# MiloszKrajewski/lz4net

Measured on AMD Instinct MI355X. Metric: uncompressed GB/s, batched 64KiB-block encode+decode: value = decode (known output size) per step over the whole resident batch; fast encode and LZ4HC encode of the same data in roofline_encode / roofline_hc, higher is better.
Workload: dtype u8

## Files before the change

### lz4net_amd/csrc/lz4hip_decode_lane4.hpp

```cpp
#pragma once
#include "lz4hip_common.hpp"
#include <type_traits>

#ifndef LZ4HIP_ITERATION_HOOK
#define LZ4HIP_ITERATION_HOOK(lane) ((void)0)
#endif
#ifndef LZ4HIP_STAT
#define LZ4HIP_STAT(slot, cond) ((void)0)
#endif
#ifdef LZ4HIP_SECTION_MARKERS
#define LZ4HIP_SECTION(name) asm volatile("; @@SECTION " name)
#elif !defined(LZ4HIP_SECTION)
#define LZ4HIP_SECTION(name) ((void)0)
#endif
#ifndef LZ4HIP_SECTION_BEGIN
#define LZ4HIP_SECTION_BEGIN() ((void)0)
#define LZ4HIP_SECTION_END(lane) ((void)0)
#endif

namespace lz4hip {

#if defined(__HIP_DEVICE_COMPILE__)
#define L4_MOV(...) wv::mov_mask(__VA_ARGS__)
#define L4_MOV8(m_, d_, a_, b_)                                                                                          \
    do {                                                                                                                 \
        wv::u32x2 p0_ = { (d_)[0], (d_)[1] }, p1_ = { (d_)[2], (d_)[3] }, p2_ = { (d_)[4], (d_)[5] }, p3_ = { (d_)[6], (d_)[7] }; \
        wv::mov2_mask(m_, p0_, wv::u32x2{ (a_).x, (a_).y }, p1_, wv::u32x2{ (a_).z, (a_).w }, p2_, wv::u32x2{ (b_).x, (b_).y }, p3_, wv::u32x2{ (b_).z, (b_).w }); \
        (d_)[0] = p0_.x; (d_)[1] = p0_.y; (d_)[2] = p1_.x; (d_)[3] = p1_.y; (d_)[4] = p2_.x; (d_)[5] = p2_.y; (d_)[6] = p3_.x; (d_)[7] = p3_.y; \
    } while (0)
#define L4_TREE_LOW(m2_, m1_, t_)                                                                                        \
    do {                                                                                                                 \
        wv::u32x2 p0_ = { (t_)[0], (t_)[1] }, p1_ = { (t_)[2], (t_)[3] }, p2_ = { (t_)[4], (t_)[5] }, p3_ = { (t_)[6], (t_)[7] }; \
        wv::mov2_mask(m2_, p0_, p1_, p1_, p2_, p2_, p3_);                                                                \
        wv::shift_dword_mask(m1_, p0_, p1_, p2_);                                                                        \
        (t_)[0] = p0_.x; (t_)[1] = p0_.y; (t_)[2] = p1_.x; (t_)[3] = p1_.y; (t_)[4] = p2_.x;                             \
    } while (0)
#else
LZ4HIP_DEVICE void lane4_mov_sel(wv::mask_t) {}
template <class T, class... REST>
LZ4HIP_DEVICE void lane4_mov_sel(wv::mask_t m, T& d, T s, REST&&... rest)
{
    d = (T)wv::sel(m, (uint32_t)s, (uint32_t)d);
    lane4_mov_sel(m, static_cast<REST&&>(rest)...);
}
#define L4_MOV(...) lane4_mov_sel(__VA_ARGS__)
#define L4_MOV8(m_, d_, a_, b_)                                                                                          \
    lane4_mov_sel(m_, (d_)[0], (uint32_t)(a_).x, (d_)[1], (uint32_t)(a_).y, (d_)[2], (uint32_t)(a_).z, (d_)[3], (uint32_t)(a_).w, \
                      (d_)[4], (uint32_t)(b_).x, (d_)[5], (uint32_t)(b_).y, (d_)[6], (uint32_t)(b_).z, (d_)[7], (uint32_t)(b_).w)
#define L4_TREE_LOW(m2_, m1_, t_)                                                                                        \
    do {                                                                                                                 \
// ... 37 lines not shown
    constexpr bool LS = (POL & 16) != 0;
    constexpr int kDual = (POL & 32) ? 0 : (LZ4HIP_DEC4_DUAL_STORE);
    static_assert(!LS || P == 32, "sector input feeds 32-byte pieces");
    constexpr int SK = LS ? 64 : P;
    constexpr int NW = 4 + P / 4, NL = LS ? 4 : P / 16;
    constexpr int HPR = FU / 16, RECS_PER_STORE = 64 / HPR;
    constexpr int kFlushRecs = (LZ4HIP_DEC4_FLUSH_RECS) ? (LZ4HIP_DEC4_FLUSH_RECS) : FS * RECS_PER_STORE;
    constexpr bool kLineNoWrap = R % 64 == 0;
    constexpr int kNearMax = R - 20;
    constexpr bool kMoves = WAVES == 1;
    unsigned char* const frec_base = lds + kRingBytes + (uint32_t)wave * 256u;
    auto frec = [&](int i) -> Aligned16* {
        if (kFlushRecs <= 16) return (Aligned16*)(frec_base + (uint32_t)i * 16u);
        return (Aligned16*)(frec_base + (uint32_t)(i >> 4) * kRow + (uint32_t)(i & 15) * 16u);
    };
    const uint32_t lane4 = (uint32_t)(wave * 64 + lane) << 2;

    auto ring_add = [](uint32_t a, uint32_t rows256) -> uint32_t {
        const uint32_t t = a + rows256;
        if (RPOW2) return t & (kRingBytes - 1u);
        const uint32_t u = t - kRingBytes;
        return u < t ? u : t;
    };
#define L4_RING(a) (*(uint32_t*)(lds + (a)))
#define L4_PHASE_SEL(p_) wv::alignbyte(0x07060504u, 0x03020100u, (uint32_t)(p_) & 3u)

    int skew = 0, in_total = 0;
    uint64_t src_al = 0;
    uint32_t out_limit = 0;
    int ip = 0;
    uint32_t W[NW];
    wv::u32x4 L[NL];
    int wb = -16;
    int lvalid = 0;
    int pend_a = 0, pend_b = 0;
    int op = 0, fl = 0;
    uint32_t oa = lane4;
    int kind = kK4None, rem = 0, off = 8;
    int gready = 0;
    int pv = 0, p_ll = 0, p_st = 0, p_ml = 0, p_off = 0, p_flags = 0, p_res = 0;
    uint32_t p_l0 = 0, p_l1 = 0, p_l2 = 0;
    int hdr = 0;
    uint32_t token = 0;
    int final_seen = 0, final_run = 0, result = 0, done = 0;
    int exhausted = 0;
    wv::u32x4 fa = { 0, 0, 0, 0 }, fb = { 0, 0, 0, 0 };
#if defined(LZ4HIP_DEC4_BALLAST_VALU) || defined(LZ4HIP_DEC4_BALLAST_LDS)
    uint32_t ballast = 0;
#endif
#pragma unroll
    for (int j = 0; j < NW; j++) W[j] = 0;
#pragma unroll
    for (int j = 0; j < NL; j++) L[j] = wv::u32x4{ 0, 0, 0, 0 };
    auto start_block = [&](bool act) {
        skew = (int)((uint64_t)src & (uint64_t)(SK - 1));
        src_al = (uint64_t)src - (uint64_t)skew;
        in_total = iend > 0 ? (int)(((int64_t)skew + iend + P - 1) & ~(int64_t)(P - 1)) : 0;
        out_limit = oend > kLastLiterals ? (uint32_t)(oend - kLastLiterals) : 0u;
        ip = 0; wb = -16 - P; lvalid = 0; pend_a = 0; pend_b = 0; op = 0; fl = 0; oa = lane4;
        kind = kK4None; rem = 0; off = 8; gready = 0;
        pv = 0; p_ll = 0; p_st = 0; p_ml = 0; p_off = 0; p_flags = 0; p_res = 0; hdr = 0; token = 0;
        final_seen = 0; final_run = 0; result = 0; done = 0;
        if (!act || (!KNOWN && iend == 0)) { done = 1; final_seen = 1; }
    };
    start_block(active);
    LZ4HIP_SECTION_BEGIN();

#define L4_STORE2(OFF_, v_) do { const uint32_t w_ = (v_); wv::lds_store_drop<OFF_>(lds, kLdsBytes, oa, w_); wv::lds_store_drop<OFF_>(lds, kLdsBytes, ob_, w_); } while (0)
#define L4_APPEND(d0_, d1_, d2_, d3_, n_, FOUR_)                                                         \
    do {                                                                                                \
        const uint32_t sb_ = (uint32_t)op & 3u;                                                         \
        const uint32_t s_ = wv::alignbyte(0x08070605u, 0x04030201u, sb_ ^ 3u);                          \
        wv::lds_mskor(&L4_RING(oa), 0xFFFFFFFFu << (8u * sb_), wv::perm(d0_, 0u, s_));                  \
        if (kDual) {                                                                                    \
                                                    \
            const uint32_t ob_ = oa - kRingBytes;                                                       \
            const uint32_t w1_ = wv::perm(d1_, d0_, s_), w2_ = wv::perm(d2_, d1_, s_);                  \
            if (kDual == 2) {                                         \
                wv::lds_store2_rows_drop<1 * WAVES, 2 * WAVES>(lds, kLdsBytes, oa, w1_, w2_);           \
                wv::lds_store2_rows_drop<1 * WAVES, 2 * WAVES>(lds, kLdsBytes, ob_, w1_, w2_);          \
                if (FOUR_) {                                                                            \
                    const uint32_t w3_ = wv::perm(d3_, d2_, s_), w4_ = wv::perm(0u, d3_, s_);           \
                    wv::lds_store2_rows_drop<3 * WAVES, 4 * WAVES>(lds, kLdsBytes, oa, w3_, w4_);       \
                    wv::lds_store2_rows_drop<3 * WAVES, 4 * WAVES>(lds, kLdsBytes, ob_, w3_, w4_);      \
                } else {                                                                                \
                    L4_STORE2(3 * kRow, wv::perm(0u, d2_, s_));                                         \
                }                                                                                       \
            } else {                                                                                    \
                L4_STORE2(kRow, w1_);                                                                   \
                L4_STORE2(2 * kRow, w2_);                                                               \
                if (FOUR_) {                                                                            \
                    L4_STORE2(3 * kRow, wv::perm(d3_, d2_, s_));                                        \
                    L4_STORE2(4 * kRow, wv::perm(0u, d3_, s_));                                         \
                } else {                                                                                \
                    L4_STORE2(3 * kRow, wv::perm(0u, d2_, s_));                                         \
                }                                                                                       \
            }                                                                                           \
        } else {                                                                                        \
            const uint32_t a1_ = ring_add(oa, kRow), a2_ = ring_add(oa, 2 * kRow), a3_ = ring_add(oa, 3 * kRow); \
            L4_RING(a1_) = wv::perm(d1_, d0_, s_);                                                      \
            L4_RING(a2_) = wv::perm(d2_, d1_, s_);                                                      \
            if (FOUR_) {                                                                                \
                L4_RING(a3_) = wv::perm(d3_, d2_, s_);                                                  \
                L4_RING(ring_add(oa, 4 * kRow)) = wv::perm(0u, d3_, s_);                                \
            } else {                                                                                    \
                L4_RING(a3_) = wv::perm(0u, d2_, s_);                                                   \
            }                                                                                           \
        }                                                                                               \
        oa = ring_add(oa, (((sb_ + (uint32_t)(n_)) << 6) & 0x700u) * (uint32_t)WAVES);                  \
        op += (n_);                                                                                     \
    } while (0)

    auto iteration = [&](auto flush_tag, wv::u32x4& ldF, wv::u32x4& usF, int& ld_pend, int& us_pend) __attribute__((always_inline)) -> bool {
        constexpr bool FLUSH = decltype(flush_tag)::value;
        constexpr bool INPUT = IE == 1 || !FLUSH;
        constexpr int kVm = (FLUSH ? FS : 0) + 1 + (INPUT ? NL : 0);
        LZ4HIP_ITERATION_HOOK(lane);
        LZ4HIP_SECTION("T2a flush records");
        bool go = false;
        int cnt = 0;
        wv::mask_t f_act_m[FS];
        Aligned16 f_rec[FS];
        uint64_t f_g[FS];
        uint32_t f_q[FS][4];
        if constexpr (FLUSH) {
            const bool need = (done == 0) & (op - fl >= FU);
            const uint64_t needy = wv::ballot(need);
            const int cnt_all = wv::popc64(needy);
            go = cnt_all != 0;
            bool mine = false;
            if (go) {
                cnt = cnt_all < kFlushRecs ? cnt_all : kFlushRecs;
                const int frank = wv::rank_below(needy);
                mine = need & (frank < kFlushRecs);
                if (mine) {
                    const uint64_t dp = (uint64_t)dst;
                    *frec(frank) = Aligned16{ { ring_add(oa, kRingBytes - ((((uint32_t)(op - fl)) << 6) & ~0xFFu) * (uint32_t)WAVES), (uint32_t)fl, (uint32_t)dp, (uint32_t)(dp >> 32) } };
                }
                fl += mine ? FU : 0;
            }
            LZ4HIP_STAT(3, need); LZ4HIP_STAT(4, need & !mine);
        }
        LZ4HIP_SECTION("T2b record read");
        if constexpr (FLUSH) {
            if (go) wv::mem_sync();
#pragma unroll
            for (int s = 0; s < FS; s++) {
                const int idx = s * RECS_PER_STORE + lane / HPR;
                f_act_m[s] = wv::cond(idx < cnt);
                f_rec[s] = *frec(idx);
            }
        }
        LZ4HIP_SECTION("T1c near-match reads");
        const uint32_t offn = kind == kK4Near ? (uint32_t)off : 4u;
        uint32_t r0, r1, r2, r3, r4;
        {
            const uint32_t back = (((offn + 3u - ((uint32_t)op & 3u)) << 6) & ~0xFFu) * (uint32_t)WAVES;
            uint32_t sa;
            if (RPOW2) sa = (oa - back) & (kRingBytes - 1u);
            else { const uint32_t t = oa - back, u = t + kRingBytes; sa = u < t ? u : t; }
            r0 = L4_RING(sa); r1 = L4_RING(ring_add(sa, kRow)); r2 = L4_RING(ring_add(sa, 2 * kRow));
            r3 = L4_RING(ring_add(sa, 3 * kRow)); r4 = L4_RING(ring_add(sa, 4 * kRow));
        }
        LZ4HIP_SECTION("T1a window refill");
        int d = ip + skew - wb;
        {
            const bool no_more = wb + 16 + P >= in_total;
            const bool cross = (d >= P) & ((lvalid != 0) | no_more);
            const wv::mask_t cm = wv::cond(d >= P) & (wv::cond(lvalid != 0) | wv::cond(no_more));
            if constexpr (LS && kMoves) {
                const bool hi_half = ((wb + 16 + P) & 32) != 0;
                const wv::mask_t hm = wv::cond(((wb + 16 + P) & 32) != 0);
                L4_MOV(cm, W[0], W[8], W[1], W[9], W[2], W[10], W[3], W[11]);
                L4_MOV8(cm & ~hm, W + 4, L[0], L[1]);
                L4_MOV8(cm & hm, W + 4, L[2], L[3]);
                lvalid = (cross & hi_half) ? 0 : lvalid;
            } else if constexpr (LS) {
#pragma unroll
                for (int j = 0; j < 4; j++) W[j] = wv::sel(cm, W[P / 4 + j], W[j]);
                const bool hi_half = ((wb + 16 + P) & 32) != 0;
                const wv::mask_t hm = wv::cond(((wb + 16 + P) & 32) != 0);
#pragma unroll
                for (int j = 0; j < 2; j++) {
                    W[4 + 4 * j] = wv::sel(cm, wv::sel(hm, L[2 + j].x, L[j].x), W[4 + 4 * j]); W[5 + 4 * j] = wv::sel(cm, wv::sel(hm, L[2 + j].y, L[j].y), W[5 + 4 * j]);
                    W[6 + 4 * j] = wv::sel(cm, wv::sel(hm, L[2 + j].z, L[j].z), W[6 + 4 * j]); W[7 + 4 * j] = wv::sel(cm, wv::sel(hm, L[2 + j].w, L[j].w), W[7 + 4 * j]);
                }
                lvalid = (cross & hi_half) ? 0 : lvalid;
            } else {
#pragma unroll
                for (int j = 0; j < 4; j++) W[j] = wv::sel(cm, W[P / 4 + j], W[j]);
#pragma unroll
                for (int j = 0; j < NL; j++) {
                    W[4 + 4 * j] = wv::sel(cm, L[j].x, W[4 + 4 * j]); W[5 + 4 * j] = wv::sel(cm, L[j].y, W[5 + 4 * j]);
                    W[6 + 4 * j] = wv::sel(cm, L[j].z, W[6 + 4 * j]); W[7 + 4 * j] = wv::sel(cm, L[j].w, W[7 + 4 * j]);
                }
                lvalid = cross ? 0 : lvalid;
            }
            wb += cross ? P : 0;
            d -= cross ? P : 0;
        }
        LZ4HIP_SECTION("T1b cursor view (select tree + rotation)");
        const bool staged16 = d < P;
        LZ4HIP_STAT(0, true); LZ4HIP_STAT(1, done == 0); LZ4HIP_STAT(2, (done == 0) & !staged16);
        uint32_t x0, x1, x2, x3;
        {
            const uint32_t k = (uint32_t)d >> 2;
            uint32_t t[NW];
            if constexpr (kMoves && P == 32) {
                const wv::mask_t m = wv::cond((k & 4u) != 0u);
#pragma unroll
                for (int j = 0; j < 8; j++) t[j] = wv::sel(m, W[j + 4], W[j]);
                L4_TREE_LOW(wv::cond((k & 2u) != 0u), wv::cond((k & 1u) != 0u), t);
            } else {
#pragma unroll
                for (int j = 0; j < NW; j++) t[j] = W[j];
                int n = NW;
#pragma unroll
                for (int sh = P / 8; sh >= 1; sh >>= 1) {
                    const wv::mask_t m = wv::cond((k & (uint32_t)sh) != 0u);
                    n -= sh;
#pragma unroll
                    for (int j = 0; j < NW; j++)
                        if (j < n) t[j] = wv::sel(m, t[j + sh], t[j]);
                }
            }
            const uint32_t sx = L4_PHASE_SEL(d);
            x0 = wv::perm(t[1], t[0], sx); x1 = wv::perm(t[2], t[1], sx); x2 = wv::perm(t[3], t[2], sx); x3 = wv::perm(t[4], t[3], sx);
        }
        LZ4HIP_SECTION("T1c near-match source rows");
        uint32_t v0, v1, v2, v3;
        {
            const uint32_t sr = L4_PHASE_SEL((uint32_t)op - offn);
            v0 = wv::perm(r1, r0, sr); v1 = wv::perm(r2, r1, sr); v2 = wv::perm(r3, r2, sr); v3 = wv::perm(r4, r3, sr);
        }

        LZ4HIP_SECTION("T3 chunk size");
        const bool room = op - fl <= R - 46;
        const bool near = kind == kK4Near, lit = kind == kK4Lit;
        const bool can = room & (rem > 0) & !((kind == kK4Far) & (gready == 0)) & !(lit & !staged16);
        const int stride = (near & (off < 16)) ? off : 16;
        int n = can ? (rem < stride ? rem : stride) : 0;
        n = ((kind == kK4Zero) & (n > 8)) ? 8 : n;
        LZ4HIP_STAT(5, (done == 0) & (rem > 0)); LZ4HIP_STAT(6, (done == 0) & (rem > 0) & (n == 0)); LZ4HIP_STAT(7, (done == 0) & (rem > 0) & !room);
        LZ4HIP_STAT(8, (done == 0) & (rem > 0) & (kind == kK4Far) & (gready == 0)); LZ4HIP_STAT(9, (done == 0) & (rem > n));
        const int rem_after = rem - n;
        const int op_end = op + rem;

        LZ4HIP_SECTION("T2c ring rows");
        if constexpr (FLUSH) {
            const int sub = lane % HPR;
#pragma unroll
            for (int s = 0; s < FS; s++) {
                const Aligned16 r = f_rec[s];
                f_g[s] = ((uint64_t)r.w[2] | ((uint64_t)r.w[3] << 32)) + (uint64_t)(r.w[1] + 16u * (uint32_t)sub);
                const uint32_t b0 = wv::sel(f_act_m[s], ring_add(r.w[0], 4u * kRow * (uint32_t)sub), lane4);
                if (kLineNoWrap) { f_q[s][0] = L4_RING(b0); f_q[s][1] = L4_RING(b0 + kRow); f_q[s][2] = L4_RING(b0 + 2 * kRow); f_q[s][3] = L4_RING(b0 + 3 * kRow); }
                else { f_q[s][0] = L4_RING(b0); f_q[s][1] = L4_RING(ring_add(b0, kRow)); f_q[s][2] = L4_RING(ring_add(b0, 2 * kRow)); f_q[s][3] = L4_RING(ring_add(b0, 3 * kRow)); }
            }
        }

        LZ4HIP_SECTION("T4 parse ahead");
        const bool may_parse = (pv == 0) & (final_seen == 0) & !(lit & (rem > 0)) & staged16;
        LZ4HIP_STAT(10, may_parse); LZ4HIP_STAT(11, (done == 0) & (pv != 0));
        if (may_parse) {
            const uint32_t tok = hdr ? token : (x0 & 255u);
            const uint32_t t4 = tok >> 4, b1 = (x0 >> 8) & 255u, mlc = tok & 15u;
            const bool e1 = (hdr == 0) & (t4 == 15u), e2 = mlc == 15u;
            const int ll = hdr ? 0 : (int)t4 + (e1 ? (int)b1 : 0);
            const bool in_win = (hdr != 0) | (t4 <= 11u);
            const int o = hdr ? 0 : 1 + (int)t4;
            uint32_t ot;
            {
                const uint32_t q = (uint32_t)o >> 2;
                const wv::mask_t m1 = wv::cond((q & 1u) != 0u), m2 = wv::cond((q & 2u) != 0u);
                const uint32_t lo = wv::sel(m2, wv::sel(m1, x3, x2), wv::sel(m1, x1, x0));
                const uint32_t hi = wv::sel(m2, x3, wv::sel(m1, x2, x1));
                ot = wv::alignbyte(hi, lo, (uint32_t)o & 3u);
            }
            const int vo = (int)(ot & 0xFFFFu);
            const uint32_t extb = (ot >> 16) & 255u;
            const int ml = (int)mlc + kMinMatch + (e2 ? (int)extb : 0);
            const int lit_end = op_end + ll;
            const int p_after = ip + o + 2;
            bool trap = (ip + 16 > iend) | (e1 & (b1 == 255u)) | (ip + 1 + (e1 ? 1 : 0) + ll > iend);
            trap |= in_win & ((e2 & (extb == 255u)) | (vo > lit_end) | ((uint32_t)lit_end + (uint32_t)ml > out_limit));
            if (KNOWN) trap |= (hdr == 0) & (lit_end > oend - 8);
            else       trap |= ((hdr == 0) & ((lit_end > oend - kMfLimit) | (ip + 1 + (e1 ? 1 : 0) + ll > iend - 8))) | (in_win & e2 & !(p_after < iend - (kLastLiterals + 1)));
            p_l0 = wv::alignbyte(x1, x0, 1); p_l1 = wv::alignbyte(x2, x1, 1); p_l2 = wv::alignbyte(x3, x2, 1);
            token = tok;
            p_ll = in_win ? ll : 0;
            p_st = in_win ? 0 : ll;
            p_ml = in_win ? ml : 0;
            p_off = vo;
            p_flags = in_win ? 0 : (int)kF4Header;
            const int ip_fast = in_win ? p_after + (e2 ? 1 : 0) : ip + 1 + (e1 ? 1 : 0);
            if (trap) {
// ... 22 lines not shown
                        if (KNOWN && err == 0 && pos + l > iend) err = -pos;
                        p_flags = kF4Header;
                    }
                    ip = pos;
                } else {
                    int p = ip;
                    const int o_ = (int)((p < iend ? src[p] : 0u) | ((p + 1 < iend ? src[p + 1] : 0u) << 8));
                    p += 2;
                    int m = (int)(token & 15u);
                    if (m == 15) {
                        if (KNOWN) {
                            uint32_t b;
                            while ((b = (p < iend ? src[p] : 0u)) == 255) { m += 255; p++; if (m > (1 << 30)) { err = -p; break; } }
                            m += (int)b; p++;
                        } else {
                            while (p < iend - (kLastLiterals + 1)) { const uint32_t b = src[p]; p++; m += (int)b; m = m > (1 << 30) ? (1 << 30) : m; if (b != 255) break; }
                        }
                    }
                    m += kMinMatch;
                    if (err != 0) {}
                    else if (op_end - o_ < 0) err = -(ip + 2);
                    else if ((int64_t)op_end + m > (int64_t)oend - kLastLiterals) err = -p;
                    p_ll = 0; p_st = 0; p_ml = m; p_off = o_; p_flags = 0;
                    ip = p;
                    hdr = 0;
                }
                if (err != 0) { p_flags = kF4Err; p_res = err; }
                hdr = (p_flags & kF4Header) ? 1 : 0;
            } else {
                ip = ip_fast;
                hdr = in_win ? 0 : 1;
            }
            LZ4HIP_SECTION("T4 parse ahead");
            pv = 1;
        }

        LZ4HIP_SECTION("T2d flush stores");
        if constexpr (FLUSH) {
#pragma unroll
            for (int s = 0; s < FS; s++) wv::vm_store16_mask(f_act_m[s], f_g[s], f_q[s][0], f_q[s][1], f_q[s][2], f_q[s][3]);
            if (go) wv::mem_sync();
        }

        LZ4HIP_SECTION("T5 far fetch");
        {
            const wv::mask_t m_rem0 = wv::cond(rem_after == 0);
            const wv::mask_t f_cont = wv::cond(kind == kK4Far) & ~m_rem0;
            const wv::mask_t f_first = m_rem0 & wv::cond(op - fl <= R - 46) & wv::cond(pv != 0) & wv::cond(p_ml != 0) & wv::cond(p_flags == 0) & wv::cond(p_off > kNearMax);
            const int f_pos = (int)wv::sel(f_cont, (uint32_t)(op + n - off), (uint32_t)(op_end + p_ll - p_off));
            const wv::mask_t f_want = f_cont | f_first;
            const wv::mask_t f_do = f_want & wv::cond(f_pos + 16 <= fl);
            wv::vm_load16_mask<POL & 3>(f_do, (uint64_t)dst + (uint64_t)(uint32_t)f_pos, ldF);
            gready = (int)wv::sel(f_do, 1u, 0u);
            LZ4HIP_STAT(15, gready != 0); LZ4HIP_STAT(16, wv::sel(f_want & ~f_do, 1u, 0u) != 0u);
        }

        LZ4HIP_SECTION("T6 input request");
        if constexpr (INPUT) {
            const int lpos = wb + 16 + P;
            const wv::mask_t req = wv::cond((done | lvalid | us_pend) == 0) & wv::cond(lpos < in_total);
            const uint64_t g = src_al + (uint64_t)(uint32_t)lpos;
            wv::vm_load16_mask_off<(POL >> 2) & 3, 0>(req, g, L[0]);
            wv::vm_load16_mask_off<(POL >> 2) & 3, 16>(req, g, L[1]);
            if constexpr (NL == 4) {
                wv::vm_load16_mask_off<(POL >> 2) & 3, 32>(req, g, L[2]);
                wv::vm_load16_mask_off<(POL >> 2) & 3, 48>(req, g, L[3]);
            }
            ld_pend = (int)wv::sel(req, 1u, 0u);
        } else {
            ld_pend = 0;
        }

        LZ4HIP_SECTION("B1 wait");
        wv::vm_wait_list<kVm>(usF, L);
        if constexpr (kMoves) lvalid |= us_pend;
        else lvalid = us_pend ? 1 : lvalid;
        us_pend = 0;

#if defined(LZ4HIP_DEC4_BALLAST_VALU) || defined(LZ4HIP_DEC4_BALLAST_LDS)
#ifdef LZ4HIP_DEC4_BALLAST_VALU
#pragma unroll
        for (int bi = 0; bi < LZ4HIP_DEC4_BALLAST_VALU; bi++) asm volatile("v_add_u32 %0, %0, %1" : "+v"(ballast) : "v"(lane4));
#endif
#ifdef LZ4HIP_DEC4_BALLAST_LDS
#pragma unroll
        for (int bi = 0; bi < LZ4HIP_DEC4_BALLAST_LDS; bi++) wv::lds_store_drop<0>(lds, kLdsBytes, 0x80000000u + lane4, ballast);
#endif
#endif
        LZ4HIP_SECTION("B3 chunk append");
        {
            if constexpr (kMoves) {
                L4_MOV(wv::cond(kind == kK4Lit), v0, x0, v1, x1, v2, x2, v3, x3);
                L4_MOV(wv::cond(kind == kK4Far), v0, (uint32_t)usF.x, v1, (uint32_t)usF.y, v2, (uint32_t)usF.z, v3, (uint32_t)usF.w);
            } else {
                const bool far_src = kind == kK4Far;
                v0 = lit ? x0 : (far_src ? usF.x : v0);
                v1 = lit ? x1 : (far_src ? usF.y : v1);
                v2 = lit ? x2 : (far_src ? usF.z : v2);
                v3 = lit ? x3 : (far_src ? usF.w : v3);
            }
            if ((kind == kK4Zero) & (n > 0)) {
                uint64_t acc = 0;
                for (int b = 0; b < n; b++) acc |= (uint64_t)dst[op + b] << (8 * b);
                v0 = (uint32_t)acc; v1 = (uint32_t)(acc >> 32);
            }
            ip += lit ? n : 0;
            L4_APPEND(v0, v1, v2, v3, n, true);
            rem = rem_after;
            off = (near & (off < 16) & (n > 0)) ? off * 2 : off;
            kind = rem == 0 ? (int)kK4None : kind;
        }

        LZ4HIP_SECTION("B4 promote + literal append");
        {
            const bool promote = (rem == 0) & (pv != 0) & room;
            LZ4HIP_STAT(12, promote); LZ4HIP_STAT(13, (done == 0) & (rem == 0) & (pv != 0) & !room); LZ4HIP_STAT(14, (done == 0) & (rem == 0) & (pv == 0));
            const bool perr = promote & ((p_flags & kF4Err) != 0);
            const bool pgo = promote & !perr;
            L4_APPEND(p_l0, p_l1, p_l2, 0u, pgo ? p_ll : 0, false);
            if (perr) {
                done = 1; final_seen = 1; final_run = 0; result = p_res;
            }
            if (pgo) {
                const bool streamed = p_st > 0;
                rem = streamed ? p_st : p_ml;
                off = streamed ? off : p_off;
                kind = streamed ? (int)kK4Lit : (p_ml == 0 ? (int)kK4None : (p_off == 0 ? (int)kK4Zero : (p_off <= kNearMax ? (int)kK4Near : (int)kK4Far)));
                final_run = (p_flags & kF4Final) ? 1 : final_run;
                result = (p_flags & kF4Final) ? p_res : result;
            }
            pv = promote ? 0 : pv;
        }

        LZ4HIP_SECTION("B5 end of block + loop");
        if (final_run && rem == 0 && !pv && !done) {
            uint32_t qa = ring_add(oa, kRingBytes - ((((uint32_t)(op - fl)) << 6) & ~0xFFu) * (uint32_t)WAVES);
            while (op - fl >= 4) { const uint32_t qd = L4_RING(qa); __builtin_memcpy(dst + fl, &qd, 4); fl += 4; qa = ring_add(qa, kRow); }
            if (fl < op) {
                const uint32_t qd = L4_RING(qa);
                for (int b = 0; fl + b < op; b++) dst[fl + b] = (uint8_t)(qd >> (8 * b));
            }
            done = 1;
        }
        return !wv::any(done == 0);
    };

    for (;;) {
        if (!std::remove_reference<NEXT>::type::kPersistent) {
            if (iteration(std::true_type{}, fa, fb, pend_a, pend_b)) break;
            if (iteration(std::integral_constant<bool, FE == 1>{}, fb, fa, pend_b, pend_a)) break;
        } else {
            (void)iteration(std::true_type{}, fa, fb, pend_a, pend_b);
            (void)iteration(std::integral_constant<bool, FE == 1>{}, fb, fa, pend_b, pend_a);
            const bool fin = (done != 0) & (exhausted == 0);
            if (wv::any(fin)) {
                if (fin) {
                    if (next(result, src, iend, dst, oend)) start_block(true);
                    else exhausted = 1;
                }
                if (!wv::any(exhausted == 0)) break;
            }
        }
    }
    LZ4HIP_SECTION_END(lane);
    return result;
#undef L4_RING
#undef L4_PHASE_SEL
#undef L4_APPEND
#undef L4_STORE2
}

__global__ void __launch_bounds__(256) count_selected_kernel(Batch b, int filter, unsigned* count)
{
    unsigned mine = 0;
    for (int64_t blk = (int64_t)blockIdx.x * 256 + threadIdx.x; blk < b.n_blocks; blk += (int64_t)gridDim.x * 256)
        mine += block_selected(filter, batch_src_len(b, blk), batch_dst_cap(b, blk)) ? 1u : 0u;
    const unsigned total = wv::scan_add(mine);
    if ((threadIdx.x & 63u) == 63u && total) atomicAdd(count, total);
}
LZ4HIP_DEVICE bool lane4_gate_open(const unsigned* gate, int gate_mode, unsigned threshold)
{
    if (gate_mode == 0) return true;
    const unsigned c = wv::uniform(*gate);
    return gate_mode == 1 ? c >= threshold : c < threshold;
}

// ... 105 lines not shown
```

### lz4net_amd/csrc/lz4hip_wave.hpp

```cpp
#pragma once
#include <hip/hip_runtime.h>
#include <stdint.h>

#define LZ4HIP_WAVE_API 1
#define LZ4HIP_DEVICE __device__ __forceinline__
#define LZ4HIP_DYN_LDS(name) extern __shared__ __attribute__((aligned(16))) unsigned char name[]
#define LZ4HIP_STATIC_LDS(name, bytes) __shared__ __attribute__((aligned(16))) unsigned char name[bytes]
#define LZ4HIP_KEEP(x) asm volatile("" : "+v"(x))

namespace wv {

constexpr int kWave = 64;

LZ4HIP_DEVICE int lane() { return (int)(threadIdx.x & 63u); }
LZ4HIP_DEVICE int wave_in_block() { return __builtin_amdgcn_readfirstlane((int)(threadIdx.x >> 6)); }

LZ4HIP_DEVICE uint32_t uniform(uint32_t v) { return (uint32_t)__builtin_amdgcn_readfirstlane((int)v); }
LZ4HIP_DEVICE int32_t uniform(int32_t v) { return __builtin_amdgcn_readfirstlane(v); }
LZ4HIP_DEVICE uint64_t uniform(uint64_t v)
{
    uint32_t lo = uniform((uint32_t)v), hi = uniform((uint32_t)(v >> 32));
    return ((uint64_t)hi << 32) | lo;
}
LZ4HIP_DEVICE int64_t uniform(int64_t v) { return (int64_t)uniform((uint64_t)v); }
// ... 87 lines not shown
    else LZ4HIP_VM_LOAD("");
#undef LZ4HIP_VM_LOAD
}
LZ4HIP_DEVICE void vm_store16_pred(bool pred, uint64_t addr, uint32_t a, uint32_t b, uint32_t c, uint32_t d)
{
    const uint64_t m = __builtin_amdgcn_ballot_w64(pred);
    uint64_t saved;
    const u32x4 v = { a, b, c, d };
    asm volatile("s_and_saveexec_b64 %[sv], %[m]\n\tglobal_store_dwordx4 %[a], %[d], off\n\ts_mov_b64 exec, %[sv]"
                 : [sv] "=&s"(saved) : [a] "v"(addr), [d] "v"(v), [m] "s"(m) : "memory");
}
template <int N>
LZ4HIP_DEVICE void vm_wait(u32x4& a, u32x4& b)
{
    static_assert(N >= 0 && N < 64, "vmcnt is a 6-bit counter");
    asm volatile("s_waitcnt vmcnt(%[n])" : "+v"(a), "+v"(b) : [n] "n"(N) : "memory");
}

template <int N, int M>
LZ4HIP_DEVICE void vm_wait_list(u32x4& a, u32x4 (&l)[M])
{
    static_assert(N >= 0 && N < 64, "vmcnt is a 6-bit counter");
    asm volatile("s_waitcnt vmcnt(%[n])" : "+v"(a) : [n] "n"(N) : "memory");
#pragma unroll
    for (int j = 0; j < M; j++) asm volatile("" : "+v"(l[j]));
}

struct mask_t { uint64_t v; };
LZ4HIP_DEVICE mask_t cond(bool p) { return mask_t{ __builtin_amdgcn_ballot_w64(p) }; }
LZ4HIP_DEVICE mask_t operator&(mask_t a, mask_t b) { return mask_t{ a.v & b.v }; }
LZ4HIP_DEVICE mask_t operator|(mask_t a, mask_t b) { return mask_t{ a.v | b.v }; }
LZ4HIP_DEVICE mask_t operator~(mask_t a) { return mask_t{ ~a.v }; }
LZ4HIP_DEVICE bool any(mask_t m) { return m.v != 0ull; }
LZ4HIP_DEVICE uint32_t sel(mask_t m, uint32_t a, uint32_t b)
{
    uint32_t r;
    asm("v_cndmask_b32_e64 %0, %1, %2, %3" : "=v"(r) : "v"(b), "v"(a), "s"(m.v));
    return r;
}
#define LZ4HIP_MM_D(i) T& d##i, T s##i
#define LZ4HIP_MM_I(i) "v_mov_b32 %[d" #i "], %[s" #i "]\n\t"
#define LZ4HIP_MM_O(i) [d##i] "+v"(d##i)
#define LZ4HIP_MM_S(i) [s##i] "v"(s##i)
#define LZ4HIP_MM_ASM(INSTRS, OUTS, INS)                                                                                          \
    static_assert(sizeof(T) == 4, "32-bit moves");                                                                                \
    uint64_t saved;                                                                                                               \
    asm volatile("s_and_saveexec_b64 %[sv], %[m]\n\t" INSTRS "s_mov_b64 exec, %[sv]" : OUTS, [sv] "=&s"(saved) : INS, [m] "s"(m.v) : "scc")
#define LZ4HIP_C ,
template <class T> LZ4HIP_DEVICE void mov_mask(mask_t m, LZ4HIP_MM_D(0), LZ4HIP_MM_D(1), LZ4HIP_MM_D(2), LZ4HIP_MM_D(3))
{ LZ4HIP_MM_ASM(LZ4HIP_MM_I(0) LZ4HIP_MM_I(1) LZ4HIP_MM_I(2) LZ4HIP_MM_I(3), LZ4HIP_MM_O(0) LZ4HIP_C LZ4HIP_MM_O(1) LZ4HIP_C LZ4HIP_MM_O(2) LZ4HIP_C LZ4HIP_MM_O(3),
                LZ4HIP_MM_S(0) LZ4HIP_C LZ4HIP_MM_S(1) LZ4HIP_C LZ4HIP_MM_S(2) LZ4HIP_C LZ4HIP_MM_S(3)); }
template <class T> LZ4HIP_DEVICE void mov_mask(mask_t m, LZ4HIP_MM_D(0), LZ4HIP_MM_D(1), LZ4HIP_MM_D(2), LZ4HIP_MM_D(3), LZ4HIP_MM_D(4), LZ4HIP_MM_D(5), LZ4HIP_MM_D(6), LZ4HIP_MM_D(7))
{ LZ4HIP_MM_ASM(LZ4HIP_MM_I(0) LZ4HIP_MM_I(1) LZ4HIP_MM_I(2) LZ4HIP_MM_I(3) LZ4HIP_MM_I(4) LZ4HIP_MM_I(5) LZ4HIP_MM_I(6) LZ4HIP_MM_I(7),
                LZ4HIP_MM_O(0) LZ4HIP_C LZ4HIP_MM_O(1) LZ4HIP_C LZ4HIP_MM_O(2) LZ4HIP_C LZ4HIP_MM_O(3) LZ4HIP_C LZ4HIP_MM_O(4) LZ4HIP_C LZ4HIP_MM_O(5) LZ4HIP_C LZ4HIP_MM_O(6) LZ4HIP_C LZ4HIP_MM_O(7),
                LZ4HIP_MM_S(0) LZ4HIP_C LZ4HIP_MM_S(1) LZ4HIP_C LZ4HIP_MM_S(2) LZ4HIP_C LZ4HIP_MM_S(3) LZ4HIP_C LZ4HIP_MM_S(4) LZ4HIP_C LZ4HIP_MM_S(5) LZ4HIP_C LZ4HIP_MM_S(6) LZ4HIP_C LZ4HIP_MM_S(7)); }
typedef uint32_t u32x2 __attribute__((ext_vector_type(2)));
LZ4HIP_DEVICE void mov2_mask(mask_t m, u32x2& d0, u32x2 s0, u32x2& d1, u32x2 s1, u32x2& d2, u32x2 s2, u32x2& d3, u32x2 s3)
{
    uint64_t saved;
    asm volatile("s_and_saveexec_b64 %[sv], %[m]\n\t"
                 "v_pk_mov_b32 %[d0], %[s0], %[s0] op_sel:[0,1]\n\tv_pk_mov_b32 %[d1], %[s1], %[s1] op_sel:[0,1]\n\t"
                 "v_pk_mov_b32 %[d2], %[s2], %[s2] op_sel:[0,1]\n\tv_pk_mov_b32 %[d3], %[s3], %[s3] op_sel:[0,1]\n\t"
                 "s_mov_b64 exec, %[sv]"
                 : [d0] "+v"(d0), [d1] "+v"(d1), [d2] "+v"(d2), [d3] "+v"(d3), [sv] "=&s"(saved)
                 : [s0] "v"(s0), [s1] "v"(s1), [s2] "v"(s2), [s3] "v"(s3), [m] "s"(m.v) : "scc");
}
// ... 92 lines not shown
```

Before: 1046.

## Keep per-lane decode state flags as wave-wide SGPR masks in non-persistent decoder

In the non-persistent lane4 decoder, per-lane boolean state (done, pending loads, literal-valid, sequence-pending, far-ready, match kind) is now held as 64-bit wave masks in scalar registers instead of per-lane integers in VGPRs. Updates become scalar mask AND/OR operations, and a lane reads its own flag through inverse_ballot. The aim is to cut VGPR pressure and the vector compare and select work around the hot loop. The cost is extra scalar instructions and mask-to-lane conversions, plus a second code path that must stay in sync with the original.

Measured after the change: 1086 (median of 6 runs). 3.8% higher.

```diff
diff --git a/lz4net_amd/csrc/lz4hip_decode_lane4.hpp b/lz4net_amd/csrc/lz4hip_decode_lane4.hpp
--- a/lz4net_amd/csrc/lz4hip_decode_lane4.hpp
+++ b/lz4net_amd/csrc/lz4hip_decode_lane4.hpp
@@ -16,6 +16,13 @@
 #ifndef LZ4HIP_SECTION_BEGIN
 #define LZ4HIP_SECTION_BEGIN() ((void)0)
 #define LZ4HIP_SECTION_END(lane) ((void)0)
+#endif
+
+#ifndef LZ4HIP_WAVE_LANE_MASKS
+namespace wv {
+LZ4HIP_DEVICE bool lane(mask_t m) { return sel(m, 1u, 0u) != 0u; }
+LZ4HIP_DEVICE mask_t mask_assign(mask_t m, mask_t when, mask_t value) { return (m & ~when) | (value & when); }
+}
 #endif
 
 namespace lz4hip {
@@ -119,17 +126,25 @@
     uint32_t W[NW];
     wv::u32x4 L[NL];
     int wb = -16;
+    constexpr bool kFlagMasks = !std::remove_reference<NEXT>::type::kPersistent;
+    const wv::mask_t kNone = wv::cond(false);
     int lvalid = 0;
     int pend_a = 0, pend_b = 0;
+    wv::mask_t lvalid_m = kNone, pend_a_m = kNone, pend_b_m = kNone;
     int op = 0, fl = 0;
     uint32_t oa = lane4;
     int kind = kK4None, rem = 0, off = 8;
+    wv::mask_t near_m = kNone, lit_m = kNone, far_m = kNone, zero_m = kNone;
     int gready = 0;
-    int pv = 0, p_ll = 0, p_st = 0, p_ml = 0, p_off = 0, p_flags = 0, p_res = 0;
+    wv::mask_t gready_m = kNone;
+    int pv = 0;
+    wv::mask_t pv_m = kNone;
+    int p_ll = 0, p_st = 0, p_ml = 0, p_off = 0, p_flags = 0, p_res = 0;
     uint32_t p_l0 = 0, p_l1 = 0, p_l2 = 0;
     int hdr = 0;
     uint32_t token = 0;
     int final_seen = 0, final_run = 0, result = 0, done = 0;
+    wv::mask_t final_run_m = kNone, done_m = kNone;
     int exhausted = 0;
     wv::u32x4 fa = { 0, 0, 0, 0 }, fb = { 0, 0, 0, 0 };
 #if defined(LZ4HIP_DEC4_BALLAST_VALU) || defined(LZ4HIP_DEC4_BALLAST_LDS)
@@ -151,6 +166,7 @@
         if (!act || (!KNOWN && iend == 0)) { done = 1; final_seen = 1; }
     };
     start_block(active);
+    if constexpr (kFlagMasks) done_m = wv::cond(done != 0);
     LZ4HIP_SECTION_BEGIN();
 
 #define L4_STORE2(OFF_, v_) do { const uint32_t w_ = (v_); wv::lds_store_drop<OFF_>(lds, kLdsBytes, oa, w_); wv::lds_store_drop<OFF_>(lds, kLdsBytes, ob_, w_); } while (0)
@@ -198,11 +214,15 @@
         op += (n_);                                                                                     \
     } while (0)
 
-    auto iteration = [&](auto flush_tag, wv::u32x4& ldF, wv::u32x4& usF, int& ld_pend, int& us_pend) __attribute__((always_inline)) -> bool {
+    auto iteration = [&](auto flush_tag, wv::u32x4& ldF, wv::u32x4& usF, int& ld_pend, int& us_pend, wv::mask_t& ld_pend_m, wv::mask_t& us_pend_m) __attribute__((always_inline)) -> bool {
         constexpr bool FLUSH = decltype(flush_tag)::value;
         constexpr bool INPUT = IE == 1 || !FLUSH;
         constexpr int kVm = (FLUSH ? FS : 0) + 1 + (INPUT ? NL : 0);
         LZ4HIP_ITERATION_HOOK(lane);
+        [[maybe_unused]] auto is_done = [&]() -> bool { if constexpr (kFlagMasks) return wv::lane(done_m); else return done != 0; };
+        [[maybe_unused]] auto has_seq = [&]() -> bool { if constexpr (kFlagMasks) return wv::lane(pv_m); else return pv != 0; };
+        [[maybe_unused]] auto is_kind = [&](int k, wv::mask_t m) -> bool { if constexpr (kFlagMasks) return wv::lane(m); else return kind == k; };
+        [[maybe_unused]] auto far_ready = [&]() -> bool { if constexpr (kFlagMasks) return wv::lane(gready_m); else return gready != 0; };
         LZ4HIP_SECTION("T2a flush records");
         bool go = false;
         int cnt = 0;
@@ -211,7 +231,9 @@
         uint64_t f_g[FS];
         uint32_t f_q[FS][4];
         if constexpr (FLUSH) {
-            const bool need = (done == 0) & (op - fl >= FU);
+            bool need;
+            if constexpr (kFlagMasks) need = !wv::lane(done_m) & (op - fl >= FU);
+            else need = (done == 0) & (op - fl >= FU);
             const uint64_t needy = wv::ballot(need);
             const int cnt_all = wv::popc64(needy);
             go = cnt_all != 0;
@@ -239,7 +261,9 @@
             }
         }
         LZ4HIP_SECTION("T1c near-match reads");
-        const uint32_t offn = kind == kK4Near ? (uint32_t)off : 4u;
+        uint32_t offn;
+        if constexpr (kFlagMasks) offn = wv::lane(near_m) ? (uint32_t)off : 4u;
+        else offn = kind == kK4Near ? (uint32_t)off : 4u;
         uint32_t r0, r1, r2, r3, r4;
         {
             const uint32_t back = (((offn + 3u - ((uint32_t)op & 3u)) << 6) & ~0xFFu) * (uint32_t)WAVES;
@@ -253,15 +277,23 @@
         int d = ip + skew - wb;
         {
             const bool no_more = wb + 16 + P >= in_total;
-            const bool cross = (d >= P) & ((lvalid != 0) | no_more);
-            const wv::mask_t cm = wv::cond(d >= P) & (wv::cond(lvalid != 0) | wv::cond(no_more));
+            wv::mask_t cm;
+            bool cross;
+            if constexpr (kFlagMasks) {
+                cm = wv::cond(d >= P) & (lvalid_m | wv::cond(no_more));
+                cross = wv::lane(cm);
+            } else {
+                cross = (d >= P) & ((lvalid != 0) | no_more);
+                cm = wv::cond(d >= P) & (wv::cond(lvalid != 0) | wv::cond(no_more));
+            }
             if constexpr (LS && kMoves) {
                 const bool hi_half = ((wb + 16 + P) & 32) != 0;
                 const wv::mask_t hm = wv::cond(((wb + 16 + P) & 32) != 0);
                 L4_MOV(cm, W[0], W[8], W[1], W[9], W[2], W[10], W[3], W[11]);
                 L4_MOV8(cm & ~hm, W + 4, L[0], L[1]);
                 L4_MOV8(cm & hm, W + 4, L[2], L[3]);
-                lvalid = (cross & hi_half) ? 0 : lvalid;
+                if constexpr (kFlagMasks) lvalid_m = lvalid_m & ~(cm & hm);
+                else lvalid = (cross & hi_half) ? 0 : lvalid;
             } else if constexpr (LS) {
 #pragma unroll
                 for (int j = 0; j < 4; j++) W[j] = wv::sel(cm, W[P / 4 + j], W[j]);
@@ -272,7 +304,8 @@
                     W[4 + 4 * j] = wv::sel(cm, wv::sel(hm, L[2 + j].x, L[j].x), W[4 + 4 * j]); W[5 + 4 * j] = wv::sel(cm, wv::sel(hm, L[2 + j].y, L[j].y), W[5 + 4 * j]);
                     W[6 + 4 * j] = wv::sel(cm, wv::sel(hm, L[2 + j].z, L[j].z), W[6 + 4 * j]); W[7 + 4 * j] = wv::sel(cm, wv::sel(hm, L[2 + j].w, L[j].w), W[7 + 4 * j]);
                 }
-                lvalid = (cross & hi_half) ? 0 : lvalid;
+                if constexpr (kFlagMasks) lvalid_m = lvalid_m & ~(cm & hm);
+                else lvalid = (cross & hi_half) ? 0 : lvalid;
             } else {
 #pragma unroll
                 for (int j = 0; j < 4; j++) W[j] = wv::sel(cm, W[P / 4 + j], W[j]);
@@ -281,14 +314,15 @@
                     W[4 + 4 * j] = wv::sel(cm, L[j].x, W[4 + 4 * j]); W[5 + 4 * j] = wv::sel(cm, L[j].y, W[5 + 4 * j]);
                     W[6 + 4 * j] = wv::sel(cm, L[j].z, W[6 + 4 * j]); W[7 + 4 * j] = wv::sel(cm, L[j].w, W[7 + 4 * j]);
                 }
-                lvalid = cross ? 0 : lvalid;
+                if constexpr (kFlagMasks) lvalid_m = lvalid_m & ~cm;
+                else lvalid = cross ? 0 : lvalid;
             }
             wb += cross ? P : 0;
             d -= cross ? P : 0;
         }
         LZ4HIP_SECTION("T1b cursor view (select tree + rotation)");
         const bool staged16 = d < P;
-        LZ4HIP_STAT(0, true); LZ4HIP_STAT(1, done == 0); LZ4HIP_STAT(2, (done == 0) & !staged16);
+        LZ4HIP_STAT(0, true); LZ4HIP_STAT(1, !is_done()); LZ4HIP_STAT(2, !is_done() & !staged16);
         uint32_t x0, x1, x2, x3;
         {
             const uint32_t k = (uint32_t)d >> 2;
@@ -323,13 +357,21 @@
 
         LZ4HIP_SECTION("T3 chunk size");
         const bool room = op - fl <= R - 46;
-        const bool near = kind == kK4Near, lit = kind == kK4Lit;
-        const bool can = room & (rem > 0) & !((kind == kK4Far) & (gready == 0)) & !(lit & !staged16);
+        bool near, lit, can;
+        if constexpr (kFlagMasks) {
+            near = wv::lane(near_m); lit = wv::lane(lit_m);
+            const bool far_waits = wv::lane(far_m & ~gready_m);
+            can = room & (rem > 0) & !far_waits & !(lit & !staged16);
+        } else {
+            near = kind == kK4Near; lit = kind == kK4Lit;
+            can = room & (rem > 0) & !((kind == kK4Far) & (gready == 0)) & !(lit & !staged16);
+        }
         const int stride = (near & (off < 16)) ? off : 16;
         int n = can ? (rem < stride ? rem : stride) : 0;
-        n = ((kind == kK4Zero) & (n > 8)) ? 8 : n;
-        LZ4HIP_STAT(5, (done == 0) & (rem > 0)); LZ4HIP_STAT(6, (done == 0) & (rem > 0) & (n == 0)); LZ4HIP_STAT(7, (done == 0) & (rem > 0) & !room);
-        LZ4HIP_STAT(8, (done == 0) & (rem > 0) & (kind == kK4Far) & (gready == 0)); LZ4HIP_STAT(9, (done == 0) & (rem > n));
+        if constexpr (kFlagMasks) n = (wv::lane(zero_m) & (n > 8)) ? 8 : n;
+        else n = ((kind == kK4Zero) & (n > 8)) ? 8 : n;
+        LZ4HIP_STAT(5, !is_done() & (rem > 0)); LZ4HIP_STAT(6, !is_done() & (rem > 0) & (n == 0)); LZ4HIP_STAT(7, !is_done() & (rem > 0) & !room);
+        LZ4HIP_STAT(8, !is_done() & (rem > 0) & is_kind(kK4Far, far_m) & !far_ready()); LZ4HIP_STAT(9, !is_done() & (rem > n));
         const int rem_after = rem - n;
         const int op_end = op + rem;
 
@@ -347,8 +389,17 @@
         }
 
         LZ4HIP_SECTION("T4 parse ahead");
-        const bool may_parse = (pv == 0) & (final_seen == 0) & !(lit & (rem > 0)) & staged16;
-        LZ4HIP_STAT(10, may_parse); LZ4HIP_STAT(11, (done == 0) & (pv != 0));
+        bool may_parse;
+        if constexpr (kFlagMasks) {
+            const wv::mask_t may_parse_m = ~pv_m & wv::cond(final_seen == 0) & ~(lit_m & wv::cond(rem > 0)) & wv::cond(staged16);
+            may_parse = wv::lane(may_parse_m);
+            LZ4HIP_STAT(11, !is_done() & has_seq());
+            pv_m = pv_m | may_parse_m;
+        } else {
+            may_parse = (pv == 0) & (final_seen == 0) & !(lit & (rem > 0)) & staged16;
+            LZ4HIP_STAT(11, !is_done() & has_seq());
+        }
+        LZ4HIP_STAT(10, may_parse);
         if (may_parse) {
             const uint32_t tok = hdr ? token : (x0 & 255u);
             const uint32_t t4 = tok >> 4, b1 = (x0 >> 8) & 255u, mlc = tok & 15u;
@@ -437,7 +488,7 @@
                 hdr = in_win ? 0 : 1;
             }
             LZ4HIP_SECTION("T4 parse ahead");
-            pv = 1;
+            if constexpr (!kFlagMasks) pv = 1;
         }
 
         LZ4HIP_SECTION("T2d flush stores");
@@ -448,22 +499,23 @@
         }
 
         LZ4HIP_SECTION("T5 far fetch");
+        const wv::mask_t m_rem0 = wv::cond(rem_after == 0);
         {
-            const wv::mask_t m_rem0 = wv::cond(rem_after == 0);
-            const wv::mask_t f_cont = wv::cond(kind == kK4Far) & ~m_rem0;
-            const wv::mask_t f_first = m_rem0 & wv::cond(op - fl <= R - 46) & wv::cond(pv != 0) & wv::cond(p_ml != 0) & wv::cond(p_flags == 0) & wv::cond(p_off > kNearMax);
+            const wv::mask_t f_cont = (kFlagMasks ? far_m : wv::cond(kind == kK4Far)) & ~m_rem0;
+            const wv::mask_t f_first = m_rem0 & wv::cond(op - fl <= R - 46) & (kFlagMasks ? pv_m : wv::cond(pv != 0)) & wv::cond(p_ml != 0) & wv::cond(p_flags == 0) & wv::cond(p_off > kNearMax);
             const int f_pos = (int)wv::sel(f_cont, (uint32_t)(op + n - off), (uint32_t)(op_end + p_ll - p_off));
             const wv::mask_t f_want = f_cont | f_first;
             const wv::mask_t f_do = f_want & wv::cond(f_pos + 16 <= fl);
             wv::vm_load16_mask<POL & 3>(f_do, (uint64_t)dst + (uint64_t)(uint32_t)f_pos, ldF);
-            gready = (int)wv::sel(f_do, 1u, 0u);
-            LZ4HIP_STAT(15, gready != 0); LZ4HIP_STAT(16, wv::sel(f_want & ~f_do, 1u, 0u) != 0u);
+            if constexpr (kFlagMasks) gready_m = f_do;
+            else gready = (int)wv::sel(f_do, 1u, 0u);
+            LZ4HIP_STAT(15, far_ready()); LZ4HIP_STAT(16, wv::sel(f_want & ~f_do, 1u, 0u) != 0u);
         }
 
         LZ4HIP_SECTION("T6 input request");
         if constexpr (INPUT) {
             const int lpos = wb + 16 + P;
-            const wv::mask_t req = wv::cond((done | lvalid | us_pend) == 0) & wv::cond(lpos < in_total);
+            const wv::mask_t req = (kFlagMasks ? ~(done_m | lvalid_m | us_pend_m) : wv::cond((done | lvalid | us_pend) == 0)) & wv::cond(lpos < in_total);
             const uint64_t g = src_al + (uint64_t)(uint32_t)lpos;
             wv::vm_load16_mask_off<(POL >> 2) & 3, 0>(req, g, L[0]);
             wv::vm_load16_mask_off<(POL >> 2) & 3, 16>(req, g, L[1]);
@@ -471,16 +523,21 @@
                 wv::vm_load16_mask_off<(POL >> 2) & 3, 32>(req, g, L[2]);
                 wv::vm_load16_mask_off<(POL >> 2) & 3, 48>(req, g, L[3]);
             }
-            ld_pend = (int)wv::sel(req, 1u, 0u);
+            if constexpr (kFlagMasks) ld_pend_m = req;
+            else ld_pend = (int)wv::sel(req, 1u, 0u);
         } else {
-            ld_pend = 0;
+            if constexpr (kFlagMasks) ld_pend_m = kNone;
+            else ld_pend = 0;
         }
 
         LZ4HIP_SECTION("B1 wait");
         wv::vm_wait_list<kVm>(usF, L);
-        if constexpr (kMoves) lvalid |= us_pend;
-        else lvalid = us_pend ? 1 : lvalid;
-        us_pend = 0;
+        if constexpr (kFlagMasks) { lvalid_m = lvalid_m | us_pend_m; us_pend_m = kNone; }
+        else {
+            if constexpr (kMoves) lvalid |= us_pend;
+            else lvalid = us_pend ? 1 : lvalid;
+            us_pend = 0;
+        }
 
 #if defined(LZ4HIP_DEC4_BALLAST_VALU) || defined(LZ4HIP_DEC4_BALLAST_LDS)
 #ifdef LZ4HIP_DEC4_BALLAST_VALU
@@ -495,16 +552,21 @@
         LZ4HIP_SECTION("B3 chunk append");
         {
             if constexpr (kMoves) {
-                L4_MOV(wv::cond(kind == kK4Lit), v0, x0, v1, x1, v2, x2, v3, x3);
-                L4_MOV(wv::cond(kind == kK4Far), v0, (uint32_t)usF.x, v1, (uint32_t)usF.y, v2, (uint32_t)usF.z, v3, (uint32_t)usF.w);
+                L4_MOV(kFlagMasks ? lit_m : wv::cond(kind == kK4Lit), v0, x0, v1, x1, v2, x2, v3, x3);
+                L4_MOV(kFlagMasks ? far_m : wv::cond(kind == kK4Far), v0, (uint32_t)usF.x, v1, (uint32_t)usF.y, v2, (uint32_t)usF.z, v3, (uint32_t)usF.w);
             } else {
-                const bool far_src = kind == kK4Far;
+                bool far_src;
+                if constexpr (kFlagMasks) far_src = wv::lane(far_m);
+                else far_src = kind == kK4Far;
                 v0 = lit ? x0 : (far_src ? usF.x : v0);
                 v1 = lit ? x1 : (far_src ? usF.y : v1);
                 v2 = lit ? x2 : (far_src ? usF.z : v2);
                 v3 = lit ? x3 : (far_src ? usF.w : v3);
             }
-            if ((kind == kK4Zero) & (n > 0)) {
+            bool zero_now;
+            if constexpr (kFlagMasks) zero_now = wv::lane(zero_m) & (n > 0);
+            else zero_now = (kind == kK4Zero) & (n > 0);
+            if (zero_now) {
                 uint64_t acc = 0;
                 for (int b = 0; b < n; b++) acc |= (uint64_t)dst[op + b] << (8 * b);
                 v0 = (uint32_t)acc; v1 = (uint32_t)(acc >> 32);
@@ -513,50 +575,89 @@
             L4_APPEND(v0, v1, v2, v3, n, true);
             rem = rem_after;
             off = (near & (off < 16) & (n > 0)) ? off * 2 : off;
-            kind = rem == 0 ? (int)kK4None : kind;
+            if constexpr (kFlagMasks) { near_m = near_m & ~m_rem0; lit_m = lit_m & ~m_rem0; far_m = far_m & ~m_rem0; zero_m = zero_m & ~m_rem0; }
+            else kind = rem == 0 ? (int)kK4None : kind;
         }
 
         LZ4HIP_SECTION("B4 promote + literal append");
         {
-            const bool promote = (rem == 0) & (pv != 0) & room;
-            LZ4HIP_STAT(12, promote); LZ4HIP_STAT(13, (done == 0) & (rem == 0) & (pv != 0) & !room); LZ4HIP_STAT(14, (done == 0) & (rem == 0) & (pv == 0));
-            const bool perr = promote & ((p_flags & kF4Err) != 0);
-            const bool pgo = promote & !perr;
-            L4_APPEND(p_l0, p_l1, p_l2, 0u, pgo ? p_ll : 0, false);
-            if (perr) {
-                done = 1; final_seen = 1; final_run = 0; result = p_res;
-            }
-            if (pgo) {
-                const bool streamed = p_st > 0;
-                rem = streamed ? p_st : p_ml;
-                off = streamed ? off : p_off;
-                kind = streamed ? (int)kK4Lit : (p_ml == 0 ? (int)kK4None : (p_off == 0 ? (int)kK4Zero : (p_off <= kNearMax ? (int)kK4Near : (int)kK4Far)));
-                final_run = (p_flags & kF4Final) ? 1 : final_run;
-                result = (p_flags & kF4Final) ? p_res : result;
-            }
-            pv = promote ? 0 : pv;
+            if constexpr (kFlagMasks) {
+                const wv::mask_t promote_m = m_rem0 & pv_m & wv::cond(room);
+                const bool promote = wv::lane(promote_m);
+                LZ4HIP_STAT(12, promote); LZ4HIP_STAT(13, !is_done() & (rem == 0) & has_seq() & !room); LZ4HIP_STAT(14, !is_done() & (rem == 0) & !has_seq());
+                const wv::mask_t perr_m = promote_m & wv::cond((p_flags & kF4Err) != 0);
+                const bool perr = wv::lane(perr_m);
+                const bool pgo = promote & !perr;
+                L4_APPEND(p_l0, p_l1, p_l2, 0u, pgo ? p_ll : 0, false);
+                if (perr) {
+                    final_seen = 1; result = p_res;
+                }
+                done_m = done_m | perr_m;
+                final_run_m = (final_run_m & ~perr_m) | (promote_m & ~perr_m & wv::cond((p_flags & kF4Final) != 0));
+                if (pgo) {
+                    const bool streamed = p_st > 0;
+                    rem = streamed ? p_st : p_ml;
+                    off = streamed ? off : p_off;
+                    result = (p_flags & kF4Final) ? p_res : result;
+                }
+                {
+                    const wv::mask_t pgo_m = promote_m & ~perr_m, st_m = wv::cond(p_st > 0);
+                    const wv::mask_t mt_m = pgo_m & ~st_m & wv::cond(p_ml != 0), nr_m = wv::cond(p_off <= kNearMax), z_m = wv::cond(p_off == 0);
+                    lit_m = lit_m | (pgo_m & st_m);
+                    zero_m = zero_m | (mt_m & z_m); near_m = near_m | (mt_m & nr_m & ~z_m); far_m = far_m | (mt_m & ~nr_m);
+                }
+                pv_m = pv_m & ~promote_m;
+            } else {
+                const bool promote = (rem == 0) & (pv != 0) & room;
+                LZ4HIP_STAT(12, promote); LZ4HIP_STAT(13, (done == 0) & (rem == 0) & (pv != 0) & !room); LZ4HIP_STAT(14, (done == 0) & (rem == 0) & (pv == 0));
+                const bool perr = promote & ((p_flags & kF4Err) != 0);
+                const bool pgo = promote & !perr;
+                L4_APPEND(p_l0, p_l1, p_l2, 0u, pgo ? p_ll : 0, false);
+                if (perr) {
+                    done = 1; final_seen = 1; final_run = 0; result = p_res;
+                }
+                if (pgo) {
+                    const bool streamed = p_st > 0;
+                    rem = streamed ? p_st : p_ml;
+                    off = streamed ? off : p_off;
+                    kind = streamed ? (int)kK4Lit : (p_ml == 0 ? (int)kK4None : (p_off == 0 ? (int)kK4Zero : (p_off <= kNearMax ? (int)kK4Near : (int)kK4Far)));
+                    final_run = (p_flags & kF4Final) ? 1 : final_run;
+                    result = (p_flags & kF4Final) ? p_res : result;
+                }
+                pv = promote ? 0 : pv;
+            }
         }
 
         LZ4HIP_SECTION("B5 end of block + loop");
-        if (final_run && rem == 0 && !pv && !done) {
+        auto exact_tail = [&]() {
             uint32_t qa = ring_add(oa, kRingBytes - ((((uint32_t)(op - fl)) << 6) & ~0xFFu) * (uint32_t)WAVES);
             while (op - fl >= 4) { const uint32_t qd = L4_RING(qa); __builtin_memcpy(dst + fl, &qd, 4); fl += 4; qa = ring_add(qa, kRow); }
             if (fl < op) {
                 const uint32_t qd = L4_RING(qa);
                 for (int b = 0; fl + b < op; b++) dst[fl + b] = (uint8_t)(qd >> (8 * b));
             }
-            done = 1;
-        }
-        return !wv::any(done == 0);
+        };
+        if constexpr (kFlagMasks) {
+            const wv::mask_t end_m = final_run_m & wv::cond(rem == 0) & ~pv_m & ~done_m;
+            if (wv::lane(end_m)) exact_tail();
+            done_m = done_m | end_m;
+            return !wv::any(~done_m);
+        } else {
+            if (final_run && rem == 0 && !pv && !done) {
+                exact_tail();
+                done = 1;
+            }
+            return !wv::any(done == 0);
+        }
     };
 
     for (;;) {
         if (!std::remove_reference<NEXT>::type::kPersistent) {
-            if (iteration(std::true_type{}, fa, fb, pend_a, pend_b)) break;
-            if (iteration(std::integral_constant<bool, FE == 1>{}, fb, fa, pend_b, pend_a)) break;
+            if (iteration(std::true_type{}, fa, fb, pend_a, pend_b, pend_a_m, pend_b_m)) break;
+            if (iteration(std::integral_constant<bool, FE == 1>{}, fb, fa, pend_b, pend_a, pend_b_m, pend_a_m)) break;
         } else {
-            (void)iteration(std::true_type{}, fa, fb, pend_a, pend_b);
-            (void)iteration(std::integral_constant<bool, FE == 1>{}, fb, fa, pend_b, pend_a);
+            (void)iteration(std::true_type{}, fa, fb, pend_a, pend_b, pend_a_m, pend_b_m);
+            (void)iteration(std::integral_constant<bool, FE == 1>{}, fb, fa, pend_b, pend_a, pend_b_m, pend_a_m);
             const bool fin = (done != 0) & (exhausted == 0);
             if (wv::any(fin)) {
                 if (fin) {
diff --git a/lz4net_amd/csrc/lz4hip_wave.hpp b/lz4net_amd/csrc/lz4hip_wave.hpp
--- a/lz4net_amd/csrc/lz4hip_wave.hpp
+++ b/lz4net_amd/csrc/lz4hip_wave.hpp
@@ -143,6 +143,9 @@
 LZ4HIP_DEVICE mask_t operator|(mask_t a, mask_t b) { return mask_t{ a.v | b.v }; }
 LZ4HIP_DEVICE mask_t operator~(mask_t a) { return mask_t{ ~a.v }; }
 LZ4HIP_DEVICE bool any(mask_t m) { return m.v != 0ull; }
+#define LZ4HIP_WAVE_LANE_MASKS 1
+LZ4HIP_DEVICE bool lane(mask_t m) { return __builtin_amdgcn_inverse_ballot_w64(m.v); }
+LZ4HIP_DEVICE mask_t mask_assign(mask_t m, mask_t when, mask_t value) { return mask_t{ (m.v & ~when.v) | (value.v & when.v) }; }
 LZ4HIP_DEVICE uint32_t sel(mask_t m, uint32_t a, uint32_t b)
 {
     uint32_t r;
```
